# williamyang98/ViterbiDecoderCpp

Hardware: AMD Instinct MI355X
Metric: decoded Mbit/s (= ACS trellis steps/s), update()+chainback(), bit-exact vs scalar reference (higher is better)
Workload: dtype u16

## Files before the change

### viterbidecodercpp_amd/csrc/common.hpp

```cpp
#pragma once
#include <stdint.h>

namespace vit {

struct DevConfig {
    uint16_t max_error, init_start, init_non_start, threshold;
    int16_t high, low;
};

__device__ __forceinline__ uint16_t abs_soft(int32_t expected, int32_t y) {
    const int16_t d = (int16_t)(expected - y);
    const int16_t n = (int16_t)(-(int32_t)d);
    return (uint16_t)(d > 0 ? d : n);
}

}
```

### viterbidecodercpp_amd/csrc/kernels_reg.hpp

```cpp
#pragma once
#include <hip/hip_runtime.h>
#include <stdint.h>

#include <type_traits>
#include <utility>

#include "common.hpp"

namespace vit {

typedef uint32_t u32;
typedef unsigned short u16x2_t __attribute__((ext_vector_type(2)));
typedef short s16x2_t __attribute__((ext_vector_type(2)));

#define VIT_DEV __device__ __forceinline__

VIT_DEV u32 pk_add(u32 a, u32 b) {
    return __builtin_bit_cast(u32, (u16x2_t)(__builtin_bit_cast(u16x2_t, a) + __builtin_bit_cast(u16x2_t, b)));
}
VIT_DEV u32 pk_sub(u32 a, u32 b) {
    return __builtin_bit_cast(u32, (u16x2_t)(__builtin_bit_cast(u16x2_t, a) - __builtin_bit_cast(u16x2_t, b)));
}
VIT_DEV u32 pk_max_s(u32 a, u32 b) {
    return __builtin_bit_cast(u32, __builtin_elementwise_max(__builtin_bit_cast(s16x2_t, a), __builtin_bit_cast(s16x2_t, b)));
// ... 922 lines not shown
                        }
                        const u32 sub = (mn ^ BIAS2) & msk;
                        static_for<NREG>([&](auto rc) __attribute__((always_inline)) {
                            constexpr int r = decltype(rc)::value;
                            m[r] = pk_sub(m[r], sub);
                        });
                        rsA += (uint64_t)((sub & 0xFFFFu) >> SHIFT);
                        rsB += (uint64_t)((sub >> 16) >> SHIFT);
                    }
                    } else
                    if (__builtin_expect(any, 0)) {
                        u32 mn = m[0];
                        static_for<NREG - 1>([&](auto rc) __attribute__((always_inline)) {
                            mn = pk_min_s(mn, m[decltype(rc)::value + 1]);
                        });
                        u32 sub;
                        if constexpr (SP::LANE_BITS) {
                            const int16_t thr = (int16_t)(uint16_t)(THRM1B2 & 0xFFFFu);
                            uint64_t tA = __builtin_amdgcn_ballot_w64((int16_t)(uint16_t)(m[0] & 0xFFFFu) > thr);
                            uint64_t tB = __builtin_amdgcn_ballot_w64((int16_t)(uint16_t)(m[0] >> 16) > thr);
                            if (a.cfg.threshold == 0) tA = tB = 0xFFFFull;
                            tA &= 0xFFFFull; tB &= 0xFFFFull;
                            tA |= tA << 16; tA |= tA << 32;
                            tB |= tB << 16; tB |= tB << 32;
                            auto s16 = __builtin_amdgcn_permlane16_swap(mn, mn, false, false);
                            mn = pk_min_s(s16[0], s16[1]);
                            auto s32 = __builtin_amdgcn_permlane32_swap(mn, mn, false, false);
                            mn = pk_min_s(s32[0], s32[1]);
                            const u32 unb = mn ^ BIAS2;
                            u32 sa, sb;
                            asm("v_cndmask_b32_e64 %0, 0, %1, %2" : "=v"(sa) : "v"(unb), "s"(tA));
                            asm("v_cndmask_b32_e64 %0, 0, %1, %2" : "=v"(sb) : "v"(unb), "s"(tB));
                            sub = (sa & 0x0000FFFFu) | (sb & 0xFFFF0000u);
                        } else {
                            const u32 need2 = pk_sub_sat_s_uniform(THRM1B2, m[0]) | FORCE;
                            const u32 msk = ((need2 & 0x8000u) ? 0x0000FFFFu : 0u) | ((need2 & 0x80000000u) ? 0xFFFF0000u : 0u);
                            sub = (mn ^ BIAS2) & msk;
                        }
#ifndef VIT_REG_FOLD
#define VIT_REG_FOLD 1
#endif
                        constexpr bool FOLD = VIT_REG_FOLD && SP::LANE_BITS != 0 && !BMCHUNK && !SPLIT && 2 * NPF < NREG;
                        bool folded = false;
                        if constexpr (FOLD) {
                            if ((!GUARDED && u + 1 < U) || t0 + (u32)u + 1u < a.t_end) {
                                static_for<NPF>([&](auto pc) __attribute__((always_inline)) {
                                    constexpr int pp = decltype(pc)::value;
                                    E[(u + 1) & 1][pp] = pk_sub(E[(u + 1) & 1][pp], sub);
                                    EB[(u + 1) & 1][pp] = pk_sub(EB[(u + 1) & 1][pp], sub);
                                });
                                folded = true;
                            }
                        }
                        if (!folded) {
                            static_for<NREG>([&](auto rc) __attribute__((always_inline)) {
                                constexpr int r = decltype(rc)::value;
                                m[r] = pk_sub(m[r], sub);
                            });
                        }
                        rsA += (uint64_t)((sub & 0xFFFFu) >> SHIFT);
                        rsB += (uint64_t)((sub >> 16) >> SHIFT);
                    }
                }
                } else if constexpr (BMCHUNK) {
                    if constexpr (u % GROUP == GROUP - 1) {
                        constexpr int Jb = u / GROUP;
                        constexpr int sl = (Jb + 1) % NG;
                        bm_produce(std::integral_constant<int, GROUP * (Jb + 1)>{}, std::integral_constant<int, sl>{});
                        load_group(t0 + (u32)(GROUP * (Jb + 1 + NG)), std::integral_constant<int, sl>{});
                    }
                    if constexpr (GENERIC) {
                        gen_chunk_row(std::integral_constant<int, u + 1>{}, std::integral_constant<int, 0>{});
                        gen_chunk_row(std::integral_constant<int, u + 1>{}, std::integral_constant<int, 1>{});
                    }
                    static_for<AHEAD>([&](auto ac) __attribute__((always_inline)) { bm_fetch_chunk(std::integral_constant<int, u + 1>{}, ac); });
                }
            }
        });
    };
    if constexpr (RESUME) {
        for (; t0 < a.t_end; t0 += U, ws_blk += (U / SPS) * 64) {
            if (t0 >= T_BEGIN && t0 + U <= a.t_end) block(std::false_type{});
            else block(std::true_type{});
        }
    } else {
        __builtin_amdgcn_s_waitcnt(0x0F70);
        for (; t0 + U <= a.t_end; t0 += U, ws_blk += (U / SPS) * 64) block(std::false_type{});
        if (t0 < a.t_end) block(std::true_type{});
    }

    if constexpr (DW != 4) {
        if (a.t_end % SPS != 0) ws_tile[(size_t)(a.t_end / SPS) * 64 + lane] = make_uint4(dq[0], dq[1], dq[2], dq[3]);
    }

    if (a.metrics_out) {
        const int ph = (int)(a.t_end % SB);
        const int lu = (int)((a.t_end + (u32)PER - 1u) % (u32)PER);
        constexpr size_t N = (size_t)1 << SB;
        static_for<NREG>([&](auto rc) __attribute__((always_inline)) {
            constexpr u32 r = decltype(rc)::value;
            const u32 x = X3 ? SP::slot3(lu, q, r) : ((q << REG_BITS) | r);
            const u32 s = ((x << ph) | (x >> (SB - ph))) & SP::SMASK;
            const u32 v = m[r] ^ BIAS2;
            if (SHIFT) {
                if (validA) ((uint8_t*)a.metrics_out)[(size_t)fA * N + s] = (uint8_t)((v & 0xFFFFu) >> 8);
                if (validB) ((uint8_t*)a.metrics_out)[(size_t)fB * N + s] = (uint8_t)(v >> 24);
            } else {
                if (validA) ((uint16_t*)a.metrics_out)[(size_t)fA * N + s] = (uint16_t)(v & 0xFFFFu);
                if (validB) ((uint16_t*)a.metrics_out)[(size_t)fB * N + s] = (uint16_t)(v >> 16);
            }
        });
    }
    if (a.renorm_sum && q == 0) {
        if (validA) a.renorm_sum[fA] = rsA;
        if (validB) a.renorm_sum[fB] = rsB;
    }
}

struct RegChainbackArgs {
    const uint4* ws;
    size_t ws_tile_stride;
    uint8_t* out;
    const u32* end_state;
    u32 frames, L;
    u32 wave_priority;
};

template <class SP>
VIT_DEV void reg_chainback_coop_body(const RegChainbackArgs& a) {
    static_assert(SP::LANE_BITS == 2 && SP::DW * SP::SPS == 4 && SP::NREG >= 32, "K = 8, 9 layout");
    constexpr int SB = SP::SB, NREG = SP::NREG, REG_BITS = SP::REG_BITS, DW = SP::DW, SPS = SP::SPS;
    constexpr int IGN = SB < 8 ? SB : 8;
    constexpr int SHIFT_STATE = 8 - IGN, SHIFT_TAIL = SB - IGN, TOTAL_BITS = SB + SHIFT_STATE;
    constexpr int PASS = 16;
    constexpr int NBUF = PASS / SPS;
    constexpr int K0 = (((7 - SB) % 8) + 8) % 8;

    const int lane = threadIdx.x & 63;
    const u32 g = lane & 15, q = lane >> 4;
    const size_t tile = blockIdx.x;
    const u32 fA_raw = (u32)tile * 32 + g, fB_raw = fA_raw + 16;
    const bool validA = fA_raw < a.frames, validB = fB_raw < a.frames;
    const u32 fA = validA ? fA_raw : a.frames - 1, fB = validB ? fB_raw : a.frames - 1;
    const uint4* rows = a.ws + tile * a.ws_tile_stride + lane;
    const size_t out_stride = ((size_t)a.L + 7) / 8;
    uint8_t* outA = a.out + (size_t)fA * out_stride;
    uint8_t* outB = a.out + (size_t)fB * out_stride;

    u32 regA = (a.end_state ? (a.end_state[fA] & SP::SMASK) : 0u) << SHIFT_STATE;
    u32 regB = (a.end_state ? (a.end_state[fB] & SP::SMASK) : 0u) << SHIFT_STATE;

    auto trace = [&](u32& reg, const uint4& v, u32 half, u32 ph1, u32 sub) __attribute__((always_inline)) {
        const u32 state = reg >> SHIFT_STATE;
        const u32 x = ((state >> ph1) | (state << (SB - ph1))) & SP::SMASK;
        const u32 qs = x >> REG_BITS, rs = x & (NREG - 1);
        const u32 pos = 32u * (u32)DW * sub + rs + (rs & ~7u) + 8u * half;
        const uint64_t lo64 = ((uint64_t)v.y << 32) | v.x, hi64 = ((uint64_t)v.w << 32) | v.z;
        const uint64_t w64 = (pos & 64u) ? hi64 : lo64;
        const u32 mine = (u32)(w64 >> (pos & 63u)) & 1u;
        const u32 bit = (u32)__shfl((int)mine, (int)(qs * 16 + g));
        reg = (reg >> 1) | (bit << (TOTAL_BITS - 1));
    };
    auto emit = [&](u32 jb) __attribute__((always_inline)) {
        if (q == 0) {
            outA[jb] = (uint8_t)((regA >> SHIFT_TAIL) & 0xFFu);
            outB[jb] = (uint8_t)((regB >> SHIFT_TAIL) & 0xFFu);
        }
    };
    auto slow_step = [&](int t) __attribute__((always_inline)) {
        const uint4 v = rows[(size_t)(t / SPS) * 64];
        const u32 ph1 = (u32)((t + 1) % SB);
        trace(regA, v, 0u, ph1, (u32)(t % SPS));
        trace(regB, v, 1u, ph1, (u32)(t % SPS));
        const int j = t - SB;
        if ((j & 7) == 0) emit((u32)j >> 3);
    };

    int t = (int)a.L - 1 + SB;
    while (t >= SB && (t & 7) != 7) slow_step(t--);
    if (t >= SB && t - (PASS - 1) >= SB) {
        uint4 buf[NBUF];
#pragma unroll
        for (int b = 0; b < NBUF; ++b) buf[b] = rows[(size_t)(t / SPS - b) * 64];
        constexpr int BPP = PASS / 8;
        constexpr int KI = 128 / BPP;
        __shared__ u32 obufA[32 * 64], obufB[32 * 64];
        typedef u32 u32_unaligned __attribute__((aligned(1)));
        u32 ph_run = (u32)((t + 1) % SB);
        while (t - (PASS - 1) >= SB) {
            __builtin_amdgcn_s_waitcnt(0x0F70);
            int it = 0;
            for (; it < KI && t - (PASS - 1) >= SB; ++it, t -= PASS) {
#pragma unroll
                for (int b = 0; b < NBUF; ++b) {
#pragma unroll
                    for (int sidx = SPS - 1; sidx >= 0; --sidx) {
                        const int k = b * SPS + (SPS - 1 - sidx);
                        const u32 ph1 = SB == 8 ? (u32)((8 - (k % 8)) % 8) : ph_run;
                        trace(regA, buf[b], 0u, ph1, (u32)sidx);
                        trace(regB, buf[b], 1u, ph1, (u32)sidx);
                        if (SB != 8) ph_run = ph_run == 0 ? SB - 1 : ph_run - 1;
                        if (k % 8 == K0) {
                            const int slot = 127 - (it * BPP + k / 8);
                            ((uint8_t*)obufA)[(slot >> 2) * 256 + lane * 4 + (slot & 3)] = (uint8_t)((regA >> SHIFT_TAIL) & 0xFFu);
                            ((uint8_t*)obufB)[(slot >> 2) * 256 + lane * 4 + (slot & 3)] = (uint8_t)((regB >> SHIFT_TAIL) & 0xFFu);
                        }
                    }
                    asm volatile("" : "+v"(regA), "+v"(regB) : : "memory");
                    const int nxt = t / SPS - b - NBUF;
                    buf[b] = rows[(size_t)(nxt < 0 ? 0 : nxt) * 64];
                    __builtin_amdgcn_sched_barrier(0);
                }
            }
            if (q == 0) {
                const int nbytes = it * BPP;
                const u32 jb_lo = (u32)(t + PASS - (K0 + 8) - SB) >> 3;
                int sl = 128 - nbytes;
                for (; (sl & 3) != 0 && sl < 128; ++sl) {
                    outA[jb_lo + (u32)(sl - (128 - nbytes))] = ((const uint8_t*)obufA)[(sl >> 2) * 256 + lane * 4 + (sl & 3)];
                    outB[jb_lo + (u32)(sl - (128 - nbytes))] = ((const uint8_t*)obufB)[(sl >> 2) * 256 + lane * 4 + (sl & 3)];
                }
                for (; sl < 128; sl += 4) {
                    *(u32_unaligned*)(outA + jb_lo + (u32)(sl - (128 - nbytes))) = obufA[(sl >> 2) * 64 + lane];
                    *(u32_unaligned*)(outB + jb_lo + (u32)(sl - (128 - nbytes))) = obufB[(sl >> 2) * 64 + lane];
                }
            }
        }
    }
    while (t >= SB) slow_step(t--);
}

#ifndef VIT_REG_CB_RING_DEPTH_K7
#define VIT_REG_CB_RING_DEPTH_K7 4
#endif
constexpr int reg_cb_ring_depth(int nreg, int R) { return nreg == 16 ? (R >= 4 ? 2 : VIT_REG_CB_RING_DEPTH_K7) : 8; }
constexpr int reg_cb_ring_flush_iters(int nreg, int R) { return (nreg == 16 && R >= 4) ? 8 : 16; }
#ifndef VIT_REG_CB_STAGGER
#define VIT_REG_CB_STAGGER 0
#endif
constexpr unsigned reg_cb_ring_slot_bytes() { return 4096u + 4u * (unsigned)VIT_REG_CB_STAGGER; }
constexpr unsigned reg_cb_ring_lds_bytes(int nreg, int R) {
    return (unsigned)reg_cb_ring_depth(nreg, R) * reg_cb_ring_slot_bytes() + (unsigned)reg_cb_ring_flush_iters(nreg, R) * 512u;
}
template <class SP>
VIT_DEV void reg_chainback_ring_body(const RegChainbackArgs& a) {
    static_assert(SP::LANE_BITS == 2 && (SP::NREG == 16 || SP::NREG == 64) && SP::DW * SP::SPS == 4 && SP::SB <= 8, "K = 7, 9 layouts");
    constexpr int SB = SP::SB, REG_BITS = SP::REG_BITS, DW = SP::DW, SPS = SP::SPS;
    constexpr int IGN = SB < 8 ? SB : 8;
    constexpr int SHIFT_STATE = 8 - IGN;
    static_assert(SB - IGN == 0, "... and its low byte is the output byte (shift_tail = 0)");
    constexpr int ITER = 32;
    constexpr int ROWS_IT = ITER / SPS;
    constexpr int D = reg_cb_ring_depth(SP::NREG, SP::R);
    static_assert(ROWS_IT % D == 0, "ring slots are compile-time constants");
    constexpr int KI = reg_cb_ring_flush_iters(SP::NREG, SP::R);
    constexpr int CT = (ITER - 1 + SB) % ITER;
    static_assert(reg_cb_ring_lds_bytes(SP::NREG, SP::R) == D * reg_cb_ring_slot_bytes() + 2 * KI * 64 * 4, "launch size of the ring kernels");
    extern __shared__ uint4 reg_cb_dyn_lds[];
    uint4* const ring = reg_cb_dyn_lds;
    u32* const obuf = (u32*)((char*)reg_cb_dyn_lds + D * reg_cb_ring_slot_bytes());
    typedef __attribute__((address_space(3))) void lds_void_t;
    typedef __attribute__((address_space(1))) const void glb_void_t;
    typedef u32 u32_unaligned __attribute__((aligned(1)));

    const int lane = threadIdx.x & 63;
    const u32 n_tiles = (a.frames + 31u) >> 5;
    const u32 jt = (u32)lane >> 4, g = (u32)lane & 15u;
    const u32 tl_raw = blockIdx.x * 4u + jt;
    const u32 tl = tl_raw < n_tiles ? tl_raw : n_tiles - 1;
    const u32 fA = tl * 32u + g < a.frames ? tl * 32u + g : a.frames - 1;
    const u32 fB = tl * 32u + g + 16u < a.frames ? tl * 32u + g + 16u : a.frames - 1;
    const size_t out_stride = ((size_t)a.L + 7) / 8;
    uint8_t* outA = a.out + (size_t)fA * out_stride;
    uint8_t* outB = a.out + (size_t)fB * out_stride;
    const uint8_t* my_rows = (const uint8_t*)(a.ws + (size_t)tl * a.ws_tile_stride);
    const u32 src_off = (u32)lane * 16u;
    const u32 pair_base = jt * (1024u + (u32)VIT_REG_CB_STAGGER) + g * 16u;

    int t = (int)a.L - 1 + SB;
    const u32 esA = a.end_state ? (a.end_state[fA] & SP::SMASK) : 0u, esB = a.end_state ? (a.end_state[fB] & SP::SMASK) : 0u;
    u32 RA = esA << (24 + SHIFT_STATE), RB = esB << (24 + SHIFT_STATE);
    u32 ph = (u32)(t + 1) % (u32)SB;
    u32 xA = ((esA >> ph) | (esA << (SB - ph))) & SP::SMASK, xB = ((esB >> ph) | (esB << (SB - ph))) & SP::SMASK;
    u32 pos = (SB - ph) % SB;

    auto byte_of = [&](u32 x, u32 base) __attribute__((always_inline)) -> u32 {
        return base + 256u * __builtin_amdgcn_ubfe(x, REG_BITS, 2) + 2u * __builtin_amdgcn_ubfe(x, 3, REG_BITS - 3);
    };
    auto step_back = [&](u32& R, u32& x, u32 byte, u32 p) __attribute__((always_inline)) {
        const u32 bit = __builtin_amdgcn_ubfe(byte, x & 7u, 1);
        R = (R >> 1) | (bit << 31);
        x = (x & ~(1u << p)) | (bit << p);
    };
    auto slow_step = [&](int tt) __attribute__((always_inline)) {
        const uint8_t* row = my_rows + (size_t)(tt / SPS) * 1024u + (u32)(tt % SPS) * (4u * DW);
        const u32 bA = row[byte_of(xA, g * 16u)], bB = row[byte_of(xB, g * 16u) + 1u];
        step_back(RA, xA, bA, pos);
        step_back(RB, xB, bB, pos);
        pos = pos == SB - 1 ? 0u : pos + 1u;
        const int j = tt - SB;
        if ((j & 7) == 0) { outA[j >> 3] = (uint8_t)(RA >> 24); outB[j >> 3] = (uint8_t)(RB >> 24); }
    };

    while (t >= SB && (t & (ITER - 1)) != CT) slow_step(t--);
    if (t - (ITER - 1) >= SB) {
        const uint8_t* tb[4];
#pragma unroll
        for (int jj = 0; jj < 4; ++jj) {
            const u32 tr = blockIdx.x * 4u + (u32)jj;
            tb[jj] = (const uint8_t*)(a.ws + (size_t)(tr < n_tiles ? tr : n_tiles - 1) * a.ws_tile_stride);
        }
        typedef __attribute__((address_space(3))) uint8_t lds_u8_t;
        u32 ring_lds = (u32)(uintptr_t)(lds_u8_t*)ring;
        asm volatile("" : "+s"(ring_lds));
        auto fill = [&](int slot, int row) __attribute__((always_inline)) {
            const u32 vo = src_off + (u32)(row < 0 ? 0 : row) * 1024u;
#pragma unroll
            for (int jj = 0; jj < 4; ++jj)
                __builtin_amdgcn_global_load_lds((glb_void_t*)(tb[jj] + vo), (lds_void_t*)(lds_u8_t*)(uintptr_t)(ring_lds + (u32)slot * reg_cb_ring_slot_bytes() + (u32)jj * (1024u + (u32)VIT_REG_CB_STAGGER)), 16, 0, 0);
        };
        constexpr int S0 = (CT / SPS) % D;
#pragma unroll
        for (int k = 0; k < D; ++k) fill((S0 - k + D) % D, t / SPS - k);
        const uint8_t* ring_b = (const uint8_t*)ring;
        while (t - (ITER - 1) >= SB) {
            __builtin_amdgcn_s_waitcnt(0x0F70);
            const int t0 = t;
            int it = 0;
            for (; it < KI && t - (ITER - 1) >= SB; ++it, t -= ITER) {
#pragma unroll
                for (int pk = 0; pk < ITER; ++pk) {
                    const int cs = CT - pk;
                    const int rk = CT / SPS - (cs >= 0 ? cs / SPS : -((-cs + SPS - 1) / SPS));
                    const int sidx = ((cs % SPS) + SPS) % SPS;
                    const int slot = ((S0 - rk) % D + D) % D;
                    constexpr int NV = 4 * (D - 1);
                    __builtin_amdgcn_s_waitcnt(0x0F70 | (NV & 15) | ((NV >> 4) << 14));
                    const u32 wA = ring_b[slot * (int)reg_cb_ring_slot_bytes() + sidx * 4 * DW + byte_of(xA, pair_base)];
                    const u32 wB = ring_b[slot * (int)reg_cb_ring_slot_bytes() + sidx * 4 * DW + 1 + byte_of(xB, pair_base)];
                    if constexpr (ITER % SB == 0) {
                        const u32 p = (u32)((SB - (((CT - pk + 1) % SB) + SB) % SB) % SB);
                        step_back(RA, xA, wA, p);
                        step_back(RB, xB, wB, p);
                    } else {
                        step_back(RA, xA, wA, pos);
                        step_back(RB, xB, wB, pos);
                        pos = pos == SB - 1 ? 0u : pos + 1u;
                    }
                    if (sidx == 0) {
                        asm volatile("" : "+v"(RA), "+v"(RB), "+v"(xA), "+v"(xB) : : "memory");
                        fill(slot, (t - pk) / SPS - D);
                        __builtin_amdgcn_sched_barrier(0);
                    }
                }
                obuf[it * 64 + lane] = __builtin_amdgcn_perm(RA, RA, 0x00010203u);
                obuf[(KI + it) * 64 + lane] = __builtin_amdgcn_perm(RB, RB, 0x00010203u);
            }
            for (int i = 0; i < it; ++i) {
                const u32 jb = (u32)(t0 - ITER * i - (ITER - 1) - SB) >> 3;
                *(u32_unaligned*)(outA + jb) = obuf[i * 64 + lane];
                *(u32_unaligned*)(outB + jb) = obuf[(KI + i) * 64 + lane];
            }
        }
        __builtin_amdgcn_s_waitcnt(0x0F70);
        if constexpr (ITER % SB == 0) pos = (SB - (u32)(t + 1) % (u32)SB) % SB;
    }
    while (t >= SB) slow_step(t--);
}

template <class SP>
VIT_DEV void reg_chainback16_body(const RegChainbackArgs& a) {
    static_assert(SP::NREG == 16 && SP::DW == 1 && SP::SPS == 4 && SP::SB == 6, "K = 7 layout");
    constexpr int SB = SP::SB;
    constexpr int IGN = SB < 8 ? SB : 8;
    constexpr int SHIFT_STATE = 8 - IGN;
    static_assert(SB - IGN == 0, "shift_tail = 0: the output byte is the 8-bit register itself");
    constexpr int NBUF = 8;

    const int lane = threadIdx.x & 63;
    const u32 n_tiles = (a.frames + 31u) >> 5;
    const u32 p_raw = blockIdx.x * 64 + lane;
    const u32 tile = (p_raw >> 4) < n_tiles ? (p_raw >> 4) : n_tiles - 1, g = p_raw & 15u;
    const u32 fA = tile * 32u + g < a.frames ? tile * 32u + g : a.frames - 1;
    const u32 fB = tile * 32u + g + 16u < a.frames ? tile * 32u + g + 16u : a.frames - 1;
    const uint4* rows = a.ws + (size_t)tile * a.ws_tile_stride + g;
    const size_t out_stride = ((size_t)a.L + 7) / 8;
    uint8_t* outA = a.out + (size_t)fA * out_stride;
    uint8_t* outB = a.out + (size_t)fB * out_stride;
    constexpr u32 SELA = 0x06040200u, SELB = 0x07050301u;

    const u32 esA = a.end_state ? (a.end_state[fA] & SP::SMASK) : 0u, esB = a.end_state ? (a.end_state[fB] & SP::SMASK) : 0u;
    u32 regA = esA << (24 + SHIFT_STATE), regB = esB << (24 + SHIFT_STATE);
    const u32 ph_top = ((u32)a.L + (u32)SB) % (u32)SB;
    u32 xA = ((esA >> ph_top) | (esA << (SB - ph_top))) & SP::SMASK, xB = ((esB >> ph_top) | (esB << (SB - ph_top))) & SP::SMASK;

    auto chase1 = [&](u32& reg, u32& x, u32 lo, u32 hi, u32 p) __attribute__((always_inline)) {
        const u32 w = x > 31u ? hi : lo;
        const u32 bit = __builtin_amdgcn_ubfe(w, x, 1);
        reg = (reg >> 1) | (bit << 31);
        x = (x & ~(1u << p)) | (bit << p);
    };
    auto chase = [&](u32 d0, u32 d1, u32 d2, u32 d3, u32 p) __attribute__((always_inline)) {
        chase1(regA, xA, __builtin_amdgcn_perm(d1, d0, SELA), __builtin_amdgcn_perm(d3, d2, SELA), p);
        chase1(regB, xB, __builtin_amdgcn_perm(d1, d0, SELB), __builtin_amdgcn_perm(d3, d2, SELB), p);
    };
    auto pos_of = [](int t) __attribute__((always_inline)) -> u32 { return (u32)((SB - (t + 1) % SB) % SB); };
    auto emit = [&](u32 jb) __attribute__((always_inline)) {
        outA[jb] = (uint8_t)(regA >> 24);
        outB[jb] = (uint8_t)(regB >> 24);
    };
    auto slow_step = [&](int t) __attribute__((always_inline)) {
        const u32* r32 = (const u32*)(rows + (size_t)(t >> 2) * 64) + (t & 3);
        chase(r32[0], r32[16 * 4], r32[32 * 4], r32[48 * 4], pos_of(t));
        const int j = t - SB;
        if ((j & 7) == 0) emit((u32)j >> 3);
    };

    int t = (int)a.L - 1 + SB;
    while (t >= SB && (((t & 3) != 3) || (((t >> 2) & 1) != 0))) slow_step(t--);
    const int g_top = t >> 2;
    const int g_min = (SB + 3) / 4;
    if (t >= SB && g_top - (NBUF - 1) >= g_min) {
        uint4 buf[NBUF][4];
#pragma unroll
        for (int b = 0; b < NBUF; ++b)
#pragma unroll
            for (int qq = 0; qq < 4; ++qq) buf[b][qq] = rows[(size_t)(g_top - b) * 64 + qq * 16];
        int gb = g_top;
        u32 pos = (u32)__builtin_amdgcn_readfirstlane((int)pos_of(4 * gb + 3));
        constexpr int KI = 32;
        __shared__ uint2 obuf[KI * 64];
        typedef u32 u32_unaligned __attribute__((aligned(1)));
        while (gb - (NBUF - 1) >= g_min) {
            __builtin_amdgcn_s_waitcnt(0x0F70);
            const int gb0 = gb;
            int it = 0;
            for (; it < KI && gb - (NBUF - 1) >= g_min; ++it, gb -= NBUF) {
                u32 accA = 0, accB = 0;
#pragma unroll
                for (int b = 0; b < NBUF; ++b) {
                    const int grp = gb - b;
#pragma unroll
                    for (int sidx = 3; sidx >= 0; --sidx) {
                        const u32 d0 = sidx == 0 ? buf[b][0].x : sidx == 1 ? buf[b][0].y : sidx == 2 ? buf[b][0].z : buf[b][0].w;
                        const u32 d1 = sidx == 0 ? buf[b][1].x : sidx == 1 ? buf[b][1].y : sidx == 2 ? buf[b][1].z : buf[b][1].w;
                        const u32 d2 = sidx == 0 ? buf[b][2].x : sidx == 1 ? buf[b][2].y : sidx == 2 ? buf[b][2].z : buf[b][2].w;
                        const u32 d3 = sidx == 0 ? buf[b][3].x : sidx == 1 ? buf[b][3].y : sidx == 2 ? buf[b][3].z : buf[b][3].w;
                        chase(d0, d1, d2, d3, pos);
                        pos = pos + 1 == (u32)SB ? 0u : pos + 1;
                        if ((b & 1) == 1 && sidx == 2) {
                            accA = (accA << 8) | (regA >> 24);
                            accB = (accB << 8) | (regB >> 24);
                        }
                    }
                    asm volatile("" : "+v"(regA), "+v"(regB), "+v"(xA), "+v"(xB) : : "memory");
                    const int nxt = grp - NBUF;
#pragma unroll
                    for (int qq = 0; qq < 4; ++qq) { typedef u32 u32x4_t __attribute__((ext_vector_type(4))); const u32x4_t v4 = __builtin_nontemporal_load((const u32x4_t*)&rows[(size_t)(nxt < 0 ? 0 : nxt) * 64 + qq * 16]); buf[b][qq] = make_uint4(v4.x, v4.y, v4.z, v4.w); }
                    __builtin_amdgcn_sched_barrier(0);
                }
                obuf[it * 64 + lane] = make_uint2(accA, accB);
            }
            for (int i = 0; i < it; ++i) {
                const uint2 v = obuf[i * 64 + lane];
                const u32 jb = (u32)((gb0 - NBUF * i) / 2 - 4);
                *(u32_unaligned*)(outA + jb) = v.x;
                *(u32_unaligned*)(outB + jb) = v.y;
            }
        }
        t = 4 * gb + 3;
    }
    while (t >= SB) slow_step(t--);
}

template <class SP>
VIT_DEV void reg_chainback0_body(const RegChainbackArgs& a) {
    static_assert(SP::LANE_BITS == 0 && SP::NREG <= 32 && (SP::DW == 1 || SP::DW == 2), "small-K layout");
    constexpr int SB = SP::SB, DW = SP::DW, SPS = SP::SPS;
    constexpr int IGN = SB < 8 ? SB : 8;
    constexpr int SHIFT_STATE = 8 - IGN, SHIFT_TAIL = SB - IGN, TOTAL_BITS = SB + SHIFT_STATE;
    constexpr int NBUF = 32 / SPS;

    const int lane = threadIdx.x & 63;
    const u32 f_raw = blockIdx.x * 64 + lane;
    const bool valid = f_raw < a.frames;
    const u32 f = valid ? f_raw : a.frames - 1;
    const u32 tile = f / SP::TILE, g = f % SP::PAIRS, half = (f % SP::TILE) / SP::PAIRS;
    const uint4* rows = a.ws + (size_t)tile * a.ws_tile_stride + g;
    const size_t out_stride = ((size_t)a.L + 7) / 8;
    uint8_t* out = a.out + (size_t)f * out_stride;
    const u32 hshift = 8u * half;

    u32 reg = (a.end_state ? (a.end_state[f] & SP::SMASK) : 0u) << SHIFT_STATE;
    auto chase = [&](u32 w0, u32 w1, u32 ph1) __attribute__((always_inline)) {
        const u32 state = reg >> SHIFT_STATE;
        const u32 x = ((state >> ph1) | (state << (SB - ph1))) & SP::SMASK;
        const u32 w = (DW == 2 && (x & 16u)) ? w1 : w0;
        const u32 bit = (w >> ((x & 7u) + hshift + 16u * ((x >> 3) & 1u))) & 1u;
        reg = (reg >> 1) | (bit << (TOTAL_BITS - 1));
    };
    auto slow_step = [&](int t) __attribute__((always_inline)) {
        const u32* r32 = (const u32*)(rows + (size_t)(t / SPS) * 64) + (t % SPS) * DW;
        chase(r32[0], DW == 2 ? r32[DW - 1] : 0u, (u32)((t + 1) % SB));
        const int j = t - SB;
        if ((j & 7) == 0) out[(u32)j >> 3] = (uint8_t)((reg >> SHIFT_TAIL) & 0xFFu);
    };

    int t = (int)a.L - 1 + SB;
    while (t >= SB && (t & 7) != 3) slow_step(t--);
    const int g_top = t / SPS;
    const int g_min = (SB + SPS - 1) / SPS;
    if (t >= SB && g_top - (NBUF - 1) >= g_min) {
        uint4 buf[NBUF];
#pragma unroll
        for (int b = 0; b < NBUF; ++b) buf[b] = rows[(size_t)(g_top - b) * 64];
        int gb = g_top;
        u32 ph = (u32)((SPS * gb + SPS - 1 + 1) % SB);
        constexpr int KI = 32;
        __shared__ u32 obuf[KI * 64];
        typedef u32 u32_unaligned __attribute__((aligned(1)));
        constexpr int K_LAST = 24 + (((3 - SB) % 8) + 8) % 8;
        while (gb - (NBUF - 1) >= g_min) {
            __builtin_amdgcn_s_waitcnt(0x0F70);
            const int gb0 = gb;
            int it = 0;
            for (; it < KI && gb - (NBUF - 1) >= g_min; ++it, gb -= NBUF) {
                u32 acc = 0;
#pragma unroll
                for (int b = 0; b < NBUF; ++b) {
#pragma unroll
                    for (int sidx = SPS - 1; sidx >= 0; --sidx) {
                        const int k = b * SPS + (SPS - 1 - sidx);
                        const int c0 = sidx * DW, c1 = sidx * DW + DW - 1;
                        const u32 w0 = c0 == 0 ? buf[b].x : c0 == 1 ? buf[b].y : c0 == 2 ? buf[b].z : buf[b].w;
                        const u32 w1 = c1 == 0 ? buf[b].x : c1 == 1 ? buf[b].y : c1 == 2 ? buf[b].z : buf[b].w;
                        chase(w0, w1, ph);
                        ph = ph == 0 ? SB - 1 : ph - 1;
                        if ((((3 - k - SB) % 8) + 8) % 8 == 0) acc = (acc << 8) | ((reg >> SHIFT_TAIL) & 0xFFu);
                    }
                    asm volatile("" : "+v"(reg) : : "memory");
                    const int nxt = gb - b - NBUF;
                    buf[b] = rows[(size_t)(nxt < 0 ? 0 : nxt) * 64];
                    __builtin_amdgcn_sched_barrier(0);
                }
                obuf[it * 64 + lane] = acc;
            }
            for (int i = 0; i < it; ++i) {
                const int t_top = SPS * (gb0 - NBUF * i) + SPS - 1;
                const u32 jb = (u32)(t_top - K_LAST - SB) >> 3;
                *(u32_unaligned*)(out + jb) = obuf[i * 64 + lane];
            }
        }
        t = SPS * gb + SPS - 1;
    }
    while (t >= SB) slow_step(t--);
}

struct RegExportArgs {
    const u32* ws32;
    size_t ws_tile_stride;
    uint64_t* out;
    u32 frames, n_steps;
};

template <class SP>
VIT_DEV void reg_export_body(const RegExportArgs& a) {
    constexpr int SB = SP::SB, NREG = SP::NREG, REG_BITS = SP::REG_BITS, DW = SP::DW, SPS = SP::SPS;
    constexpr int W = SB >= 6 ? 1 << (SB - 6) : 1;
    const size_t idx = (size_t)blockIdx.x * blockDim.x + threadIdx.x;
    const size_t total = (size_t)a.frames * a.n_steps * W;
    if (idx >= total) return;
    const u32 w = (u32)(idx % W);
    const u32 t = (u32)((idx / W) % a.n_steps);
    const u32 f = (u32)(idx / ((size_t)W * a.n_steps));
    const u32 tile = f / SP::TILE, g = f % SP::PAIRS, half = (f % SP::TILE) / SP::PAIRS;
    const int ph1 = (int)((t + 1) % SB);
    uint64_t word = 0;
    for (u32 b = 0; b < 64; ++b) {
        const u32 s = w * 64 + b;
        if (s > SP::SMASK) break;
        const u32 x = ((s >> ph1) | (s << (SB - ph1))) & SP::SMASK;
        const u32 qs = x >> REG_BITS, rs = x & (NREG - 1);
        const size_t row = (size_t)tile * a.ws_tile_stride + (size_t)(t / SPS) * 64 + qs * SP::PAIRS + g;
        const u32 dwi = (DW == 4) ? (rs >> 4) : (t % SPS) * DW + (rs >> 4);
        const u32 v = a.ws32[row * 4 + dwi];
        word |= (uint64_t)((v >> SP::dec_bit(rs, half)) & 1u) << b;
    }
    a.out[idx] = word;
}

template <class SP>
constexpr int reg_update_min_waves() { return 2; }
#define VIT_REG_UPDATE_IS_CAPPED(K, R) ((K) == 9 || ((K) == 7 && (R) == 3))
#if defined(VIT_REG_TU_K) && VIT_REG_UPDATE_IS_CAPPED(VIT_REG_TU_K, VIT_REG_TU_R)
#define VIT_REG_UPDATE_VGPR_CAP __attribute__((amdgpu_num_vgpr(120)))
#else
#define VIT_REG_UPDATE_VGPR_CAP
#endif
template <class SP, int SHIFT>
__global__ void __launch_bounds__(64, reg_update_min_waves<SP>()) VIT_REG_UPDATE_VGPR_CAP reg_update_kernel(RegUpdateArgs a) {
#ifdef VIT_REG_TU_K
    static_assert(SP::K == VIT_REG_TU_K && SP::R == VIT_REG_TU_R, "the register cap above was chosen for another code");
#endif
#ifdef VIT_HIP_CLOCK_STAMPS
    const uint64_t c0 = __builtin_amdgcn_s_memtime(), r0 = __builtin_amdgcn_s_memrealtime();
#endif
    reg_update_body<SP, SHIFT, false>(a);
#ifdef VIT_HIP_CLOCK_STAMPS
    if (a.stamps && (threadIdx.x & 63) == 0) {
        uint64_t* st = a.stamps + (size_t)blockIdx.x * 6;
        st[0] = c0; st[1] = r0; st[2] = __builtin_amdgcn_s_memtime(); st[3] = __builtin_amdgcn_s_memrealtime();
        st[4] = (uint64_t)__builtin_amdgcn_s_getreg((3 << 11) | 20);
        st[5] = (uint64_t)__builtin_amdgcn_s_getreg((31 << 11) | 4);
    }
#endif
}
template <class SP, int SHIFT>
__global__ void __launch_bounds__(64, 1) reg_resume_kernel(RegUpdateArgs a) { reg_update_body<SP, SHIFT, true>(a); }

template <class SP>
VIT_DEV void reg_chainback_body(const RegChainbackArgs& a) {
    if constexpr (SP::LANE_BITS == 0) reg_chainback0_body<SP>(a);
    else if constexpr (SP::NREG == 16) reg_chainback16_body<SP>(a);
    else if constexpr (SP::NREG == 64) reg_chainback_ring_body<SP>(a);
    else reg_chainback_coop_body<SP>(a);
}
constexpr unsigned reg_chainback_dyn_lds_bytes(int K, int R, bool alt) {
    return (K == 9 && !alt) ? reg_cb_ring_lds_bytes(64, R) : (K == 7 && alt) ? reg_cb_ring_lds_bytes(16, R) : 0u;
}
constexpr unsigned reg_chainback_frames_per_block(int K) { return (K == 7 || K == 9) ? 128u : K < 7 ? 64u : 32u; }
template <class SP>
constexpr int reg_chainback_min_waves() { return SP::NREG == 64 ? 1 : 2; }
template <class SP>
__global__ void __launch_bounds__(64, reg_chainback_min_waves<SP>()) reg_chainback_kernel(RegChainbackArgs a) {
    if (a.wave_priority) __builtin_amdgcn_s_setprio(3);
    reg_chainback_body<SP>(a);
}
template <class SP>
VIT_DEV void reg_chainback_alt_body(const RegChainbackArgs& a) {
    if constexpr (SP::NREG == 64) reg_chainback_coop_body<SP>(a);
    else if constexpr (SP::NREG == 16 && SP::LANE_BITS == 2) reg_chainback_ring_body<SP>(a);
}
template <class SP>
constexpr int reg_chainback_alt_min_waves() { return SP::NREG == 16 ? 1 : 2; }
template <class SP>
__global__ void __launch_bounds__(64, reg_chainback_alt_min_waves<SP>()) reg_chainback_alt_kernel(RegChainbackArgs a) { reg_chainback_alt_body<SP>(a); }
template <class SP>
__global__ void reg_export_kernel(RegExportArgs a) { reg_export_body<SP>(a); }

}
```

Before: 163,300.

## Pack both chainback states into one register with precomputed LDS address bits

For the K=7 register chainback, the two lanes' trellis states are stored as 16-bit halves of one packed word. Each half is laid out so its low bits form the LDS byte address directly and its high bits give the bit-select shift. Each traceback step then needs one packed shift, one v_bfi and two alignbits, instead of separate bitfield extracts, address arithmetic and masking for each state. This shortens the serial dependency chain per step. The packed path only runs when the LDS ring starts at address 0 and the layout constants match; otherwise it falls back to slow steps.

```diff
diff --git a/viterbidecodercpp_amd/csrc/common.hpp b/viterbidecodercpp_amd/csrc/common.hpp
--- a/viterbidecodercpp_amd/csrc/common.hpp
+++ b/viterbidecodercpp_amd/csrc/common.hpp
@@ -14,4 +14,35 @@
     return (uint16_t)(d > 0 ? d : n);
 }
 
+namespace cb_pk {
+typedef unsigned short u16x2 __attribute__((vector_size(4)));
+
+constexpr uint32_t ADDR_MASK = 0x0FFFu;
+constexpr uint32_t pos_bit(uint32_t p) { return p < 3u ? 12u + p : p == 3u ? 1u : 4u + p; }
+constexpr uint32_t POS_BITS = 0x981EDCu;
+constexpr uint32_t pos_mask(uint32_t p) { return 0x00010001u << pos_bit(p); }
+
+__host__ __device__ inline uint32_t pack_half(uint32_t x, uint32_t base) {
+    return base | ((x & 7u) << 12) | (((x >> 3) & 1u) << 1) | ((x >> 4) << 8);
 }
+__host__ __device__ inline uint32_t unpack_half(uint32_t h) { return ((h >> 12) & 7u) | (((h >> 1) & 1u) << 3) | (((h >> 8) & 3u) << 4); }
+__host__ __device__ inline uint32_t pack(uint32_t xA, uint32_t xB, uint32_t base) { return pack_half(xA, base) | (pack_half(xB, base) << 16); }
+__host__ __device__ inline uint32_t addr_a(uint32_t Z) { return Z & ADDR_MASK; }
+__host__ __device__ inline uint32_t addr_b(uint32_t Z) { return (Z >> 16) & ADDR_MASK; }
+
+__host__ __device__ inline uint32_t step(uint32_t Z, uint32_t W, uint32_t sh, uint32_t mask, uint32_t& bits) {
+    const u16x2 z = __builtin_bit_cast(u16x2, Z), w = __builtin_bit_cast(u16x2, W);
+    const u16x2 m = z >> 12;
+    const u16x2 b = w >> m;
+    bits = __builtin_bit_cast(uint32_t, b);
+#if defined(__HIP_DEVICE_COMPILE__)
+    uint32_t d;
+    asm("v_bfi_b32 %0, %1, %2, %3" : "=v"(d) : "s"(mask), "v"(bits << sh), "v"(Z));
+    return d;
+#else
+    return (Z & ~mask) | ((bits << sh) & mask);
+#endif
+}
+}
+
+}
diff --git a/viterbidecodercpp_amd/csrc/kernels_reg.hpp b/viterbidecodercpp_amd/csrc/kernels_reg.hpp
--- a/viterbidecodercpp_amd/csrc/kernels_reg.hpp
+++ b/viterbidecodercpp_amd/csrc/kernels_reg.hpp
@@ -1248,15 +1248,23 @@
         if ((j & 7) == 0) { outA[j >> 3] = (uint8_t)(RA >> 24); outB[j >> 3] = (uint8_t)(RB >> 24); }
     };
 
+    constexpr bool PACKED = SP::NREG == 16 && SB == 6 && REG_BITS == 4 && DW == 1 && ITER % SB != 0 && VIT_REG_CB_STAGGER == 0;
+    typedef __attribute__((address_space(3))) uint8_t lds_u8_t;
+    bool ring_ok = true;
+    if constexpr (PACKED) {
+        u32 ring_at = (u32)(uintptr_t)(lds_u8_t*)ring;
+        asm volatile("" : "+s"(ring_at));
+        ring_ok = ring_at == 0u;
+    }
+
     while (t >= SB && (t & (ITER - 1)) != CT) slow_step(t--);
-    if (t - (ITER - 1) >= SB) {
+    if (t - (ITER - 1) >= SB && ring_ok) {
         const uint8_t* tb[4];
 #pragma unroll
         for (int jj = 0; jj < 4; ++jj) {
             const u32 tr = blockIdx.x * 4u + (u32)jj;
             tb[jj] = (const uint8_t*)(a.ws + (size_t)(tr < n_tiles ? tr : n_tiles - 1) * a.ws_tile_stride);
         }
-        typedef __attribute__((address_space(3))) uint8_t lds_u8_t;
         u32 ring_lds = (u32)(uintptr_t)(lds_u8_t*)ring;
         asm volatile("" : "+s"(ring_lds));
         auto fill = [&](int slot, int row) __attribute__((always_inline)) {
@@ -1269,6 +1277,11 @@
 #pragma unroll
         for (int k = 0; k < D; ++k) fill((S0 - k + D) % D, t / SPS - k);
         const uint8_t* ring_b = (const uint8_t*)ring;
+        u32 Z = 0;
+        if constexpr (PACKED) {
+            static_assert((3u * 1024u + 15u * 16u) <= cb_pk::ADDR_MASK && ((3u * 1024u + 15u * 16u) & 0x0302u) == 0u, "the pair's piece and the slot's address bits");
+            Z = cb_pk::pack(xA, xB, pair_base);
+        }
         while (t - (ITER - 1) >= SB) {
             __builtin_amdgcn_s_waitcnt(0x0F70);
             const int t0 = t;
@@ -1281,6 +1294,24 @@
                     const int sidx = ((cs % SPS) + SPS) % SPS;
                     const int slot = ((S0 - rk) % D + D) % D;
                     constexpr int NV = 4 * (D - 1);
+                    if constexpr (PACKED) {
+                        __builtin_amdgcn_s_waitcnt(0x0F70 | (NV & 15) | ((NV >> 4) << 14));
+                        const u32 wA = *(const lds_u8_t*)(uintptr_t)(cb_pk::addr_a(Z) + (u32)(slot * (int)reg_cb_ring_slot_bytes() + sidx * 4 * DW));
+                        const u32 wB = *(const lds_u8_t*)(uintptr_t)(cb_pk::addr_b(Z) + (u32)(slot * (int)reg_cb_ring_slot_bytes() + sidx * 4 * DW + 1));
+                        const u32 W = (wB << 16) | wA;
+                        const u32 sh = (cb_pk::POS_BITS >> (4u * pos)) & 15u;
+                        u32 bits;
+                        Z = cb_pk::step(Z, W, sh, 0x00010001u << sh, bits);
+                        RA = __builtin_amdgcn_alignbit(bits, RA, 1);
+                        RB = __builtin_amdgcn_alignbit(bits >> 16, RB, 1);
+                        pos = pos == SB - 1 ? 0u : pos + 1u;
+                        if (sidx == 0) {
+                            asm volatile("" : "+v"(RA), "+v"(RB), "+v"(Z) : : "memory");
+                            fill(slot, (t - pk) / SPS - D);
+                            __builtin_amdgcn_sched_barrier(0);
+                        }
+                        continue;
+                    }
                     __builtin_amdgcn_s_waitcnt(0x0F70 | (NV & 15) | ((NV >> 4) << 14));
                     const u32 wA = ring_b[slot * (int)reg_cb_ring_slot_bytes() + sidx * 4 * DW + byte_of(xA, pair_base)];
                     const u32 wB = ring_b[slot * (int)reg_cb_ring_slot_bytes() + sidx * 4 * DW + 1 + byte_of(xB, pair_base)];
@@ -1310,6 +1341,7 @@
         }
         __builtin_amdgcn_s_waitcnt(0x0F70);
         if constexpr (ITER % SB == 0) pos = (SB - (u32)(t + 1) % (u32)SB) % SB;
+        if constexpr (PACKED) { xA = cb_pk::unpack_half(Z & 0xFFFFu); xB = cb_pk::unpack_half(Z >> 16); }
     }
     while (t >= SB) slow_step(t--);
 }
```

Measured after the change: 159,600. -2.3%, worse.
